# LeeBY68/Hier-SLAM

Measured on AMD Instinct MI355X. Metric: fwd+bwd renders/sec @1200x680, 500k Gaussians, 4-level tree; grad max-abs-err vs ref, higher is better.
Workload: dtype f32; 1 GPU; semantic fwd+bwd render, 1200x680, P=500000 slam Gaussians, K=26 semantic channels, dense upstream grads on colour/semantic/depth/median/opacity; P=500000, visible=480888, num_rendered=1136056, width=1200, height=680, K=26, parallelism=single GPU, keyframes_per_rank=1

## Files before the change

### hier-slam_amd/csrc/hsr_api.hip

```cpp
#include <stdarg.h>

#include <chrono>
#include <time.h>
#include <stdio.h>
#include <stdlib.h>
#include <string.h>

#include <mutex>
#include <type_traits>
#include <vector>

#include "../../include/hsr_rasterizer.h"
#include "hsr_tile_common.h"

namespace {

thread_local char g_err[512] = "";

template <typename T>
inline void take(char*& p, T*& out, size_t count)
{
    uintptr_t a = (reinterpret_cast<uintptr_t>(p) + 255) & ~(uintptr_t)255;
    out = reinterpret_cast<T*>(a);
    p = reinterpret_cast<char*>(out + count);
// ... 134 lines not shown
    if (d < 0 || d >= HSR_MAX_DEVICES) {
        hsr_set_error("device index %d out of range", d);
        return HSR_ERR_INVALID_ARGUMENT;
    }
    g_pc = &g_counters_by_device[d];
    if (!g_pinned) {
        HSR_HIP_CHECK(hipHostMalloc(reinterpret_cast<void**>(&g_pinned), 64, hipHostMallocPortable | hipHostMallocMapped));
        g_pinned[0] = g_pinned[1] = g_pinned[2] = 0;
        HSR_HIP_CHECK(hipHostGetDevicePointer(reinterpret_cast<void**>(&g_pinned_dev), g_pinned, 0));
    }
    return HSR_OK;
}
int read_counter_begin(const uint32_t* dev, hipStream_t stream)
{
    int rc;
    if ((rc = counter_buffer()) != HSR_OK) return rc;
    if (!g_counter_event) HSR_HIP_CHECK(hipEventCreateWithFlags(&g_counter_event, hipEventDisableTiming));
    HSR_HIP_CHECK(hipMemcpyAsync(g_pinned, dev, sizeof(uint32_t), hipMemcpyDeviceToHost, stream));
    HSR_HIP_CHECK(hipMemcpyAsync(g_pinned + 2, dev + 1, sizeof(uint32_t), hipMemcpyDeviceToHost, stream));
    HSR_HIP_CHECK(hipEventRecord(g_counter_event, stream));
    return HSR_OK;
}
thread_local double g_host_wait_ms = 0.0;
thread_local int g_last_per_tile = 0;
int read_counter_end(uint32_t* host_out)
{
    const auto t0 = std::chrono::steady_clock::now();
    HSR_HIP_CHECK(hipEventSynchronize(g_counter_event));
    g_host_wait_ms += std::chrono::duration<double, std::milli>(std::chrono::steady_clock::now() - t0).count();
    *host_out = g_pinned[0];
    return HSR_OK;
}
int poll_counter(uint32_t seq, hipStream_t stream, uint32_t* host_out, volatile uint32_t* slot = nullptr)
{
    const auto t0 = std::chrono::steady_clock::now();
    if (slot) {
        unsigned spins = 0;
        uint32_t cur;
        while ((cur = __atomic_load_n(&slot[1], __ATOMIC_ACQUIRE)) != seq) {
            if (cur != 0 && (int32_t)(cur - seq) > 0) {
                hsr_set_error("non-blocking forward: this call's num_rendered was overwritten — more than %d non-blocking forwards were "
                              "started on the device before it was resolved (resolve or drop earlier ones first)", HSR_ASYNC_SLOTS - 1);
                return HSR_ERR_INVALID_ARGUMENT;
            }
            if ((++spins & 0xFFFu) == 0) {
                const double el = std::chrono::duration<double>(std::chrono::steady_clock::now() - t0).count();
                if (el > 10.0) {
// ... 169 lines not shown
            seq = ++g_counter_seq;
            if (seq == 0) seq = ++g_counter_seq;
            slot_dev = g_pinned_dev;
        }
        StageTimer tm(HSR_STAGE_FWD_DUPLICATE, stream);
        hsr_launch_bin_count(plan, P, radii, tiles_x, tiles_y, g, bin_scratch, im.ranges, stream, slot_dev, seq);
    } else {
        StageTimer tm(HSR_STAGE_FWD_SCAN, stream);
        hsr_launch_scan_block_sums(P, g, stream);
    }
    HSR_LAUNCH_CHECK(in.debug, stream);

    if (!binned && (rc = read_counter_begin(g.counters, stream)) != HSR_OK) return rc;

    RenderFwdArgs ra;
    ra.W = W; ra.H = H; ra.K = in.semantic ? in.K : 0; ra.semantic = in.semantic;
    ra.ranges = im.ranges; ra.point_list = nullptr; ra.masks = nullptr; ra.means2D = g.means2D; ra.conic_opacity = g.conic_opacity;
    ra.depths = g.depths; ra.colors = in.colors_precomp ? in.colors_precomp : g.rgb; ra.semantics = in.semantics;
    ra.rec = g.rec;
    ra.final_T = im.final_T; ra.n_contrib = im.n_contrib; ra.median_pos = im.median_pos;
    ra.out_color = in.out_color; ra.out_semantic = in.out_semantic; ra.out_depth = in.out_depth;
    ra.out_median_depth = in.out_median; ra.out_opacity = in.out_opacity; ra.out_mask = in.out_mask;
    ra.bin = BinDevRef{nullptr, nullptr, 0};
    if (!in.semantic && !in.out_mask) {
        hsr_set_error("out_mask is NULL");
        return HSR_ERR_INVALID_ARGUMENT;
    }

    bool speculated = false;
    if (will_speculate) {
        const BinDevRef ref{static_cast<char*>(binning->ptr), reinterpret_cast<const uint32_t*>(g.counters), binning->capacity};
        BinState none{nullptr, nullptr, nullptr, nullptr, nullptr};
        {
            StageTimer tm(HSR_STAGE_FWD_DUPLICATE, stream);
            hsr_launch_bin_emit(plan, P, radii, tiles_x, tiles_y, g, bin_scratch, im.ranges, nullptr, stream, &ref);
        }
        {
            StageTimer tm(HSR_STAGE_FWD_SORT, stream);
            hsr_launch_tile_sort(none, T, P, im.ranges, stream, &ref, g_last_per_tile);
        }
        ra.bin = ref;
        {
            StageTimer tm(HSR_STAGE_FWD_RENDER, stream);
            hsr_launch_render_forward(ra, stream);
        }
        HSR_HIP_CHECK(hipGetLastError());
        speculated = true;
    }
    if (go_async) {
        ticket->seq = seq;
        ticket->device = slot_device;
        ticket->slot = slot_host;
        ticket->binning_base = static_cast<char*>(binning->ptr);
        ticket->binning_capacity = binning->capacity;
        ticket->prefiltered = in.prefiltered;
        return HSR_PENDING;
    }

    uint32_t R32 = 0;
    if ((rc = binned ? poll_counter(seq, stream, &R32) : read_counter_end(&R32)) != HSR_OK) return rc;
    if (R32 > 0x7fffffffu) {
        hsr_set_error("num_rendered %u overflows int", R32);
        return HSR_ERR_INVALID_ARGUMENT;
    }
    const int R = (int)R32;
    if (in.prefiltered && __atomic_load_n(&g_pinned[2], __ATOMIC_RELAXED) != 0) {
        hsr_set_error("Point is filtered although prefiltered is set. This shouldn't happen!");
        return HSR_ERR_INVALID_ARGUMENT;
    }
    if (speculated) {
        BinState chk;
        const BinDevRef ref{static_cast<char*>(binning->ptr), nullptr, binning->capacity};
        g_last_per_tile = R / (T > 0 ? T : 1);
        if (hsr_bin_resolve(ref, R32, &chk)) return R;
        hsr_launch_bin_count(plan, P, radii, tiles_x, tiles_y, g, bin_scratch, im.ranges, stream, g_pinned_dev, seq);
        ra.bin = BinDevRef{nullptr, nullptr, 0};
    }

    char* bptr;
    if ((rc = acquire(binning, hsr_required_binning_bytes(R), "binning", &bptr)) != HSR_OK) return rc;
    BinState b;
    hsr_carve_bin(bptr, R, &b);

    if (binned) {
        StageTimer tm(HSR_STAGE_FWD_DUPLICATE, stream);
        hsr_launch_bin_emit(plan, P, radii, tiles_x, tiles_y, g, bin_scratch, im.ranges, b.keys, stream);
    }
    if (binned) {
        HSR_LAUNCH_CHECK(in.debug, stream);
        StageTimer tm(HSR_STAGE_FWD_SORT, stream);
        if (R > 0) hsr_launch_tile_sort(b, T, P, im.ranges, stream, nullptr, R / (T > 0 ? T : 1));
    } else {
        const bool emit_sorted = hsr_sort_emit_into_sorted_buffers(end_bit);
        uint64_t* emit_k = emit_sorted ? b.keys : b.keys_unsorted;
        uint32_t* emit_v = emit_sorted ? b.vals : b.vals_unsorted;
        {
            StageTimer tm(HSR_STAGE_FWD_DUPLICATE, stream);
            BinState be = b;
            be.keys_unsorted = emit_k;
            be.vals_unsorted = emit_v;
            hsr_launch_duplicate(P, radii, tiles_x, tiles_y, g, be, im.ranges, stream);
        }
        HSR_LAUNCH_CHECK(in.debug, stream);
        StageTimer tm(HSR_STAGE_FWD_SORT, stream);
        if ((rc = hsr_launch_sort_pairs(b, R, end_bit, T, im.ranges, stream)) != HSR_OK) return rc;
    }
    HSR_LAUNCH_CHECK(in.debug, stream);

    ra.point_list = b.vals;
    ra.masks = b.vals_unsorted;
    {
        StageTimer tm(HSR_STAGE_FWD_RENDER, stream);
        hsr_launch_render_forward(ra, stream);
    }
// ... 480 lines not shown
```

### hier-slam_amd/csrc/hsr_common.h

```cpp
#pragma once
#include <hip/hip_runtime.h>
#include <stddef.h>
#include <stdint.h>

#define HSR_TILE_X 16
#define HSR_TILE_Y 16
#define HSR_TILE_PIX 256
#define HSR_NUM_CHANNELS 3

struct GeomState {
    float* depths;
    float2* means2D;
    float4* conic_opacity;
    float* cov3D;
    float* rgb;
    uint8_t* clamped;
    uint32_t* tiles_touched;
    uint32_t* point_offsets;
    int* radii;
    uint32_t* block_sums;
    uint32_t* counters;
    float4* rec;
};
struct ImgState {
// ... 68 lines not shown
    const float* colors_precomp;
    const float* viewmatrix;
    const float* projmatrix;
    const float* cam_pos;
    float tan_fovx, tan_fovy, focal_x, focal_y;
    int* radii;
    int prefiltered;
    int tiles_x, tiles_y;
};

int hsr_launch_mark_visible(int P, const float* means3D, const float* view, const float* proj, uint8_t* present,
                            hipStream_t stream);
int hsr_launch_preprocess(const PreprocessArgs& a, GeomState& g, hipStream_t stream);
int hsr_launch_scan_block_sums(int P, GeomState& g, hipStream_t stream);
int hsr_launch_duplicate(int P, const int* radii, int tiles_x, int tiles_y, GeomState& g, BinState& b, uint2* ranges,
                         hipStream_t stream);
int hsr_launch_sort_pairs(BinState& b, int R, int end_bit, int T, uint2* ranges, hipStream_t stream);
struct HsrBinPlan { int nblk, per_block; };
bool hsr_bin_plan(int P, int T, size_t scratch_words, HsrBinPlan* plan);
int hsr_launch_bin_count(const HsrBinPlan& plan, int P, const int* radii, int tiles_x, int tiles_y, GeomState& g, uint32_t* scratch,
                         uint2* ranges, hipStream_t stream, uint32_t* host_counter = nullptr, uint32_t host_seq = 0);
int hsr_launch_bin_emit(const HsrBinPlan& plan, int P, const int* radii, int tiles_x, int tiles_y, GeomState& g, const uint32_t* scratch,
                        uint2* ranges, uint64_t* comp, hipStream_t stream, const BinDevRef* ref = nullptr);
int hsr_launch_tile_sort(BinState& b, int T, int P, const uint2* ranges, hipStream_t stream, const BinDevRef* ref = nullptr,
                         int avg_per_tile_hint = 0);
int hsr_sort_tile_passes(int end_bit);
bool hsr_sort_emit_into_sorted_buffers(int end_bit);
int hsr_launch_tile_ranges(int R, int T, const uint64_t* keys, uint2* ranges, hipStream_t stream);
int hsr_launch_tile_ranges_only(int R, const uint64_t* keys, uint2* ranges, hipStream_t stream);

struct RenderFwdArgs {
    int W, H, K, semantic;
    const uint2* ranges;
    const uint32_t* point_list;
    uint32_t* masks;
    const float2* means2D;
    const float4* conic_opacity;
    const float* depths;
    const float* colors;
    const float4* rec;
    const float* semantics;
    float* final_T;
    uint32_t* n_contrib;
    uint32_t* median_pos;
    float* out_color;
    float* out_semantic;
    float* out_depth;
    float* out_median_depth;
    float* out_opacity;
    float* out_mask;
    BinDevRef bin;
};
int hsr_launch_render_forward(const RenderFwdArgs& a, hipStream_t stream);

struct RenderBwdArgs {
    int W, H, K, semantic, P;
    const float* bg;
    const uint2* ranges;
// ... 75 lines not shown
```

### hier-slam_amd/csrc/hsr_render_fwd.hip

```cpp

#include "hsr_tile_common.h"

#ifdef HSR_TRACE
__device__ unsigned long long g_hsr_trace_fwd[16384 * 8];
extern "C" int hsr_debug_read_trace_fwd(unsigned long long* host, int n)
{
    return (int)hipMemcpyFromSymbol(host, HIP_SYMBOL(g_hsr_trace_fwd), sizeof(unsigned long long) * (size_t)n);
}
#define TRF_NOW() clock64()
#define TRF_ADD(acc, t0) (acc) += (unsigned long long)(clock64() - (t0))
#else
#define TRF_NOW() 0ll
#define TRF_ADD(acc, t0) ((void)0)
#endif

namespace {

template <int W>
__device__ __forceinline__ void quad_fma_words(float (&s)[16], const float (&x)[4], float w)
{
    static_assert(W >= 1 && W <= 4, "1..4 words = 4..16 channels per block");
    if constexpr (W == 4) {
        asm("s_nop 1\n\t"
            "v_fmac_f32_dpp %0, %16, %20 quad_perm:[0,0,0,0] row_mask:0xf bank_mask:0xf\n\t"
// ... 43 lines not shown
            : "+v"(s[0]), "+v"(s[1]), "+v"(s[2]), "+v"(s[3]), "+v"(s[4]), "+v"(s[5]), "+v"(s[6]), "+v"(s[7])
            : "v"(x[0]), "v"(x[1]), "v"(w));
    } else {
        asm("s_nop 1\n\t"
            "v_fmac_f32_dpp %0, %4, %5 quad_perm:[0,0,0,0] row_mask:0xf bank_mask:0xf\n\t"
            "v_fmac_f32_dpp %1, %4, %5 quad_perm:[1,1,1,1] row_mask:0xf bank_mask:0xf\n\t"
            "v_fmac_f32_dpp %2, %4, %5 quad_perm:[2,2,2,2] row_mask:0xf bank_mask:0xf\n\t"
            "v_fmac_f32_dpp %3, %4, %5 quad_perm:[3,3,3,3] row_mask:0xf bank_mask:0xf"
            : "+v"(s[0]), "+v"(s[1]), "+v"(s[2]), "+v"(s[3])
            : "v"(x[0]), "v"(w));
    }
}

template <int KC, bool BASE, bool MASK, bool ALIGNED, bool PF = false>
__global__ void __launch_bounds__(256, KC <= 26 ? (KC == 16 ? 5 : 4) : (PF ? (KC <= 48 ? 4 : (KC <= 80 ? 3 : 2)) : 1)) render_fwd_kernel(RenderFwdArgs a, int c0)
{
    constexpr int BATCH = KC <= 32 ? (KC > 26 ? 200 : 240)
                                   : (KC <= 48 ? 152 : ((KC <= 64 || KC == 74) ? 144 : (KC <= 80 ? 136 : (KC <= 112 ? 144 : 128))));
    static_assert(KC <= 32 || PF, "batch sizes beyond 32 channels assume the touched rows (PF)");
    constexpr int RW = (KC + 2 + 3) & ~3;
    constexpr bool QS = PF && KC > 0;
    constexpr int NGF = QS ? RW / 16 : 0;
    constexpr int REM = QS ? (RW % 16) / 4 : 0;
    __shared__ float4 s_rec[BATCH * 2];
    __shared__ float4 s_row[BATCH * (RW / 4)];
    __shared__ uint8_t s_sublist[16 * HSR_SUB_LSTRIDE];
    __shared__ uint8_t s_subcnt[4][16];
    __shared__ int s_wdone[4];

    const int tile = hsr_block_tile(blockIdx.x, ((a.W + HSR_TILE_X - 1) / HSR_TILE_X) * ((a.H + HSR_TILE_Y - 1) / HSR_TILE_Y));
    if (tile >= ((a.W + HSR_TILE_X - 1) / HSR_TILE_X) * ((a.H + HSR_TILE_Y - 1) / HSR_TILE_Y)) return;
    const int t = threadIdx.x, wv = t >> 6;
    if (a.bin.base) {
        BinState bs;
        if (!hsr_bin_resolve(a.bin, *a.bin.R_dev, &bs)) {
            hsr_poison_tile(a, tile, t, BASE, c0, KC);
            return;
        }
        a.point_list = bs.vals;
        a.masks = bs.vals_unsorted;
    }
    const TileGeom tg = tile_geom_sub(tile, a.W, a.H, t);
    const bool inside = tg.inside;
    const size_t N = (size_t)a.W * a.H;
    float pfx = tg.pfx, pfy = tg.pfy;
    asm volatile("" : "+v"(pfx), "+v"(pfy));
    const float tile_x0 = (float)(tg.tx * HSR_TILE_X), tile_y0 = (float)(tg.ty * HSR_TILE_Y);

    unsigned long long tr_bar = 0, tr_stage = 0, tr_blend = 0, tr_iters = 0, tr_pub = 0;
    (void)tr_pub;
    const long long tr_t0 = TRF_NOW();
    long long tr_t1 = tr_t0;
    (void)tr_bar; (void)tr_stage; (void)tr_blend; (void)tr_iters; (void)tr_t0; (void)tr_t1;
    const uint2 range = a.ranges[tile];
    const int n = (int)(range.y - range.x);

    float T = 1.0f;
    uint32_t last_contributor = 0;
    float C0 = 0, C1 = 0, C2 = 0, Dd = 0, Mm = 0;
    uint32_t median_at = 0;
    float median_D = 15.0f;
    float S[KC > 0 ? KC : 1];
#pragma unroll
    for (int c = 0; c < (KC > 0 ? KC : 1); c++) S[c] = 0.f;
    bool done = !inside;

    int id_next = 0;
    float2 p_xy = {0, 0};
    float4 p_co = {0, 0, 0, 0};
    float p_r = 0, p_g = 0, p_b = 0, p_d = 0;
    float p_sem[(KC > 0 && !PF) ? KC : 1];
#pragma unroll
    for (int c = 0; c < ((KC > 0 && !PF) ? KC : 1); c++) p_sem[c] = 0.f;
    constexpr int NPF = PF ? (KC + 15) / 16 + 1 : 1;
    float pf_t[NPF];
#pragma unroll
    for (int c = 0; c < NPF; c++) pf_t[c] = 0.f;
    float pf_sink = 0.f;
// ... 16 lines not shown
            if (KC > 0 && PF) {
                const float* row = a.semantics + id * (size_t)a.K + c0;
                const int last = min(KC, a.K - c0) - 1;
#pragma unroll
                for (int c = 0; c < NPF; c++) pf_t[c] = row[min(16 * c, last)];
            } else if (KC > 0) {
                if (ALIGNED) {
                    const float2* row = reinterpret_cast<const float2*>(a.semantics + id * (size_t)KC);
#pragma unroll
                    for (int q = 0; q < KC / 2; q++) {
                        const float2 v = row[q];
                        p_sem[PF ? 0 : 2 * q] = v.x;
                        p_sem[PF ? 0 : 2 * q + 1] = v.y;
                    }
                } else {
                    const float* row = a.semantics + id * (size_t)a.K + c0;
#pragma unroll
                    for (int c = 0; c < KC; c++) p_sem[PF ? 0 : c] = (c0 + c < a.K) ? row[c] : 0.f;
                }
            }
        }
    };
    if (n > 0) {
        const int id0 = fetch_id(0);
        id_next = fetch_id(BATCH);
        load_record(id0);
    }
    auto resolve_median = [&](int start) {
        if (BASE && median_at > (uint32_t)start) {
            const int j = (int)median_at - 1 - start;
            constexpr int c = KC + 1;
            constexpr int pos = (QS && c / 16 < NGF) ? (16 * (c / 16) + 4 * (c % 4) + (c % 16) / 4) : c;
            median_D = reinterpret_cast<const float*>(s_row)[j * RW + pos];
        }
    };


    for (int start = 0; start < n; start += BATCH) {
        const bool wave_done = __ballot(!done) == 0ull;
        if ((t & 63) == 0) s_wdone[wv] = wave_done;
        const long long tb0 = TRF_NOW();
        (void)tb0;
        __syncthreads();
        TRF_ADD(tr_bar, tb0);
        if (start == 0) tr_t1 = TRF_NOW();
        const long long ts0 = TRF_NOW();
        (void)ts0;
        if (s_wdone[0] & s_wdone[1] & s_wdone[2] & s_wdone[3]) break;
// ... 282 lines not shown
```

### hier-slam_amd/csrc/hsr_sort.hip

```cpp
#include "hsr_common.h"

namespace {

constexpr int SORT_THREADS = 256;
constexpr int SORT_ITEMS = 16;
constexpr int SORT_TILE = SORT_THREADS * SORT_ITEMS;
static_assert(SORT_TILE == HSR_SORT_TILE, "hsr_common.h sizes the histogram scratch");

__global__ void __launch_bounds__(SORT_THREADS) sort_hist_kernel(const uint64_t* __restrict__ keys, int n, int shift,
                                                                 uint32_t mask, int nblocks, uint32_t* __restrict__ hist)
{
    __shared__ uint32_t h[256];
    h[threadIdx.x] = 0;
    __syncthreads();
    const int base = blockIdx.x * SORT_TILE;
#pragma unroll 4
    for (int i = 0; i < SORT_ITEMS; i++) {
        const int j = base + i * SORT_THREADS + threadIdx.x;
        if (j < n) atomicAdd(&h[(uint32_t)(keys[j] >> shift) & mask], 1u);
    }
    __syncthreads();
    hist[(size_t)threadIdx.x * nblocks + blockIdx.x] = h[threadIdx.x];
}

// ... 86 lines not shown
        wcnt[0][threadIdx.x] = g;
        wcnt[1][threadIdx.x] = g + c0;
        wcnt[2][threadIdx.x] = g + c0 + c1;
        wcnt[3][threadIdx.x] = g + c0 + c1 + c2;
    }
    __syncthreads();
#pragma unroll
    for (int r = 0; r < SORT_ITEMS; r++) {
        const int j = base + r * 64 + lane;
        if (j < n) {
            const uint32_t d = (uint32_t)(key[r] >> shift) & mask;
            const uint32_t pos = wcnt[w][d] + rank[r];
            kout[pos] = key[r];
            vout[pos] = val[r];
        }
    }
}

}

uint32_t hsr_sort_hist_entries(int R) { return hsr_sort_hist_entries_inline((uint32_t)(R > 0 ? R : 0)); }


constexpr int TS_MAX = 2048;

__device__ __forceinline__ void ts_block_radix(uint64_t* ka, uint32_t* va, uint64_t* kb, uint32_t* vb, int r0, int n,
                                               uint32_t* hist , uint32_t (*wcnt)[256], int gid_passes)
{
    const int t = threadIdx.x, lane = t & 63, w = t >> 6;
    const uint64_t lt = (1ull << lane) - 1ull;
    const int npass = gid_passes + 4;
    for (int pass = 0; pass < npass; pass++) {
        const bool on_gid = pass < gid_passes;
        const int shift = 8 * (on_gid ? pass : pass - gid_passes);
        hist[t] = 0;
#pragma unroll
        for (int i = 0; i < 4; i++) wcnt[i][t] = 0;
        __syncthreads();
        for (int i = t; i < n; i += 256)
            atomicAdd(&hist[((on_gid ? va[r0 + i] : (uint32_t)ka[r0 + i]) >> shift) & 255u], 1u);
        __syncthreads();
        {
            const uint32_t v = hist[t];
            uint32_t inc = v;
#pragma unroll
            for (int o = 1; o < 64; o <<= 1) {
                const uint32_t x = __shfl_up(inc, o);
                if (lane >= o) inc += x;
            }
            __shared__ uint32_t wt[4];
            if (lane == 63) wt[w] = inc;
            __syncthreads();
            uint32_t off = 0;
#pragma unroll
            for (int i = 0; i < 4; i++) off += i < w ? wt[i] : 0u;
            hist[t] = off + inc - v;
        }
        __syncthreads();
        for (int c = 0; c < n; c += 256) {
            const int i = c + t;
            const bool valid = i < n;
            const uint64_t k = valid ? ka[r0 + i] : 0ull;
            const uint32_t v = valid ? va[r0 + i] : 0u;
            const uint32_t d = ((on_gid ? v : (uint32_t)k) >> shift) & 255u;
            uint64_t m = __ballot(valid);
#pragma unroll
            for (int b = 0; b < 8; b++) {
                const bool bit = (d >> b) & 1u;
                const uint64_t bal = __ballot(bit);
                m &= bit ? bal : ~bal;
            }
            const uint32_t before = __popcll(m & lt);
            if (valid && before == 0) wcnt[w][d] = (uint32_t)__popcll(m);
            __syncthreads();
            if (valid) {
                uint32_t pos = hist[d] + before;
#pragma unroll
                for (int i2 = 0; i2 < 4; i2++) pos += i2 < w ? wcnt[i2][d] : 0u;
                kb[r0 + pos] = k;
                vb[r0 + pos] = v;
            }
            __syncthreads();
            hist[t] += wcnt[0][t] + wcnt[1][t] + wcnt[2][t] + wcnt[3][t];
#pragma unroll
            for (int i2 = 0; i2 < 4; i2++) wcnt[i2][t] = 0;
            __syncthreads();
        }
        uint64_t* tk = ka; ka = kb; kb = tk;
        uint32_t* tv = va; va = vb; vb = tv;
        __threadfence_block();
    }
    if (npass & 1) {
        __syncthreads();
        for (int i = t; i < n; i += 256) {
            kb[r0 + i] = ka[r0 + i];
            vb[r0 + i] = va[r0 + i];
        }
    }
}

constexpr int TP_MAX = 1024;
constexpr int TQ_MAX = 2048;

template <int E, int NT>
__device__ __forceinline__ void net_bitonic(uint64_t (&x)[E], int tid, ulonglong2* buf)
{
    constexpr int N = NT * E;
#pragma unroll
    for (int k = 2; k <= N; k <<= 1) {
#pragma unroll
        for (int j = k >> 1; j > 0; j >>= 1) {
            if (j < E) {
#pragma unroll
                for (int r = 0; r < E; r++) {
                    if ((r & j) == 0) {
                        const bool up = k < E ? ((r & k) == 0) : (((E * tid) & k) == 0);
                        const uint64_t a = x[r], b = x[r + j];
                        const bool sw = (a > b) == up;
                        x[r] = sw ? b : a;
                        x[r + j] = sw ? a : b;
                    }
                }
            } else {
                const int m = j / E;
                const bool cross = m >= 64;
#pragma unroll
                for (int q = 0; q < E / 2; q++) buf[q * NT + tid] = make_ulonglong2(x[2 * q], x[2 * q + 1]);
                if (cross) {
                    __syncthreads();
                } else {
                    __builtin_amdgcn_fence(__ATOMIC_RELEASE, "wavefront");
                    __builtin_amdgcn_wave_barrier();
                    __builtin_amdgcn_fence(__ATOMIC_ACQUIRE, "wavefront");
                }
                const bool keep_min = ((tid & m) == 0) == (((E * tid) & k) == 0);
#pragma unroll
                for (int q = 0; q < E / 2; q++) {
                    const ulonglong2 y = buf[q * NT + (tid ^ m)];
                    const uint64_t a0 = x[2 * q], a1 = x[2 * q + 1];
                    x[2 * q] = keep_min ? (a0 < y.x ? a0 : y.x) : (a0 > y.x ? a0 : y.x);
                    x[2 * q + 1] = keep_min ? (a1 < y.y ? a1 : y.y) : (a1 > y.y ? a1 : y.y);
                }
                if (cross) {
                    __syncthreads();
                } else {
                    __builtin_amdgcn_fence(__ATOMIC_RELEASE, "wavefront");
                    __builtin_amdgcn_wave_barrier();
                    __builtin_amdgcn_fence(__ATOMIC_ACQUIRE, "wavefront");
                }
            }
        }
    }
}

__device__ __forceinline__ void block_sort_tile(int tile, const uint2* __restrict__ ranges, uint64_t* __restrict__ keys,
                                                uint32_t* __restrict__ vals, uint64_t* __restrict__ keys_alt,
                                                uint32_t* __restrict__ vals_alt, int gid_passes, int composite_in, uint64_t* comp,
                                                uint32_t* hist, uint32_t (*wcnt)[256])
{
    const uint2 rg = ranges[tile];
    const int r0 = (int)rg.x, n = (int)(rg.y - rg.x);
    const int t = threadIdx.x;
    const uint64_t my_tile_hi = (uint64_t)tile << 32;
    if (n <= 0) return;
    if (n == 1 || n > TS_MAX) {
        if (composite_in) {
            for (int i = t; i < n; i += 256) {
                const uint64_t c = keys[r0 + i];
                keys[r0 + i] = my_tile_hi | (c >> 32);
                vals[r0 + i] = (uint32_t)c;
            }
            __syncthreads();
        }
        if (n == 1) return;
    }
    if (n > TS_MAX) {
        ts_block_radix(keys, vals, keys_alt, vals_alt, r0, n, hist, wcnt, gid_passes);
        return;
    }
    if (composite_in) {
        static_assert(TQ_MAX == TS_MAX && TS_MAX * 8 >= 4 * 256 * 16, "exchange buffer = the LDS network's key array");
        uint64_t x[8];
#pragma unroll
        for (int r = 0; r < 8; r++) {
            const int e = 8 * t + r;
            x[r] = e < n ? keys[r0 + e] : ~0ull;
        }
        net_bitonic<8, 256>(x, t, reinterpret_cast<ulonglong2*>(comp));
#pragma unroll
        for (int r = 0; r < 8; r++) {
            const int e = 8 * t + r;
            if (e < n) {
                keys[r0 + e] = my_tile_hi | (x[r] >> 32);
                vals[r0 + e] = (uint32_t)x[r];
            }
        }
        return;
    }
    int N = 64;
    while (N < n) N <<= 1;
    const uint64_t tile_hi = keys[r0] & 0xFFFFFFFF00000000ull;
    for (int i = t; i < N; i += 256)
        comp[i] = i < n ? (((keys[r0 + i] & 0xFFFFFFFFull) << 32) | (uint64_t)vals[r0 + i]) : ~0ull;
    __syncthreads();
    bool cross = false;
    for (int k = 2; k <= N; k <<= 1) {
        for (int j = k >> 1; j > 0; j >>= 1) {
            if (j >= 128 || cross) __syncthreads();
            cross = j >= 128;
            for (int i = t; i < N / 2; i += 256) {
                const int lo = ((i & ~(j - 1)) << 1) | (i & (j - 1));
                const int hi = lo | j;
                const bool up = (lo & k) == 0;
                const uint64_t a = comp[lo], b = comp[hi];
                if ((a > b) == up) {
                    comp[lo] = b;
                    comp[hi] = a;
                }
            }
        }
    }
    __syncthreads();
    for (int i = t; i < n; i += 256) {
        const uint64_t c = comp[i];
        keys[r0 + i] = tile_hi | (c >> 32);
        vals[r0 + i] = (uint32_t)c;
    }
}

__global__ void __launch_bounds__(256) tile_sort_kernel(const uint2* __restrict__ ranges, uint64_t* __restrict__ keys,
                                                        uint32_t* __restrict__ vals, uint64_t* __restrict__ keys_alt,
                                                        uint32_t* __restrict__ vals_alt, int gid_passes, int composite_in, BinDevRef ref)
{
    if (ref.base) {
        BinState bs;
        if (!hsr_bin_resolve(ref, *ref.R_dev, &bs)) return;
        keys = bs.keys; vals = bs.vals; keys_alt = bs.keys_unsorted; vals_alt = bs.vals_unsorted;
    }
    __shared__ uint64_t comp[TS_MAX];
    __shared__ uint32_t hist[256];
    __shared__ uint32_t wcnt[4][256];
    if (composite_in == 2) {
        const uint2 rg = ranges[blockIdx.x];
        if (rg.y - rg.x <= (uint32_t)TP_MAX) return;
        composite_in = 1;
    }
    block_sort_tile((int)blockIdx.x, ranges, keys, vals, keys_alt, vals_alt, gid_passes, composite_in, comp, hist, wcnt);
}

template <int E>
__device__ __forceinline__ void pair_sort_tile(int r0, int n, int tid, uint64_t tile_hi, uint64_t* __restrict__ keys,
                                               uint32_t* __restrict__ vals, ulonglong2* buf)
{
    uint64_t x[E];
#pragma unroll
    for (int r = 0; r < E; r++) {
        const int e = E * tid + r;
        x[r] = e < n ? keys[r0 + e] : ~0ull;
    }
    net_bitonic<E, 128>(x, tid, buf);
#pragma unroll
    for (int r = 0; r < E; r++) {
        const int e = E * tid + r;
        if (e < n) {
            keys[r0 + e] = tile_hi | (x[r] >> 32);
            vals[r0 + e] = (uint32_t)x[r];
        }
    }
}

__global__ void __launch_bounds__(256, 7) tile_sort_pair_kernel(int T, const uint2* __restrict__ ranges, uint64_t* __restrict__ keys,
                                                             uint32_t* __restrict__ vals, uint64_t* __restrict__ keys_alt,
                                                             uint32_t* __restrict__ vals_alt, int gid_passes, int big_too, BinDevRef ref)
{
    constexpr int RAW_WG = TS_MAX * 8 + 256 * 4 + 4 * 256 * 4, RAW_PAIR = 2 * 4 * 128 * 16;
    constexpr int RAW = RAW_WG > RAW_PAIR ? RAW_WG : RAW_PAIR;
    __shared__ __attribute__((aligned(16))) unsigned char s_raw[RAW];
    __shared__ int s_big[2];
    if (ref.base) {
        BinState bs;
        if (!hsr_bin_resolve(ref, *ref.R_dev, &bs)) return;
        keys = bs.keys; vals = bs.vals; keys_alt = bs.keys_unsorted; vals_alt = bs.vals_unsorted;
    }
    const int pair = threadIdx.x >> 7, tid = threadIdx.x & 127;
    const int tile = blockIdx.x * 2 + pair;
    int n = 0, r0 = 0;
    if (tile < T) {
        const uint2 rg = ranges[tile];
        r0 = (int)rg.x;
        n = (int)(rg.y - rg.x);
    }
    if (tid == 0) s_big[pair] = n > TP_MAX;
    {
        ulonglong2* buf = reinterpret_cast<ulonglong2*>(s_raw) + pair * (4 * 128);
        const uint64_t tile_hi = (uint64_t)tile << 32;
        if (n > 0 && n <= 256) pair_sort_tile<2>(r0, n, tid, tile_hi, keys, vals, buf);
        else if (n > 256 && n <= 512) pair_sort_tile<4>(r0, n, tid, tile_hi, keys, vals, buf);
        else if (n > 512 && n <= TP_MAX) pair_sort_tile<8>(r0, n, tid, tile_hi, keys, vals, buf);
        else { __syncthreads(); __syncthreads(); }
    }
    if (!big_too) return;
    __syncthreads();
    uint64_t* comp = reinterpret_cast<uint64_t*>(s_raw);
    uint32_t* hist = reinterpret_cast<uint32_t*>(s_raw + TS_MAX * 8);
    uint32_t (*wcnt)[256] = reinterpret_cast<uint32_t (*)[256]>(s_raw + TS_MAX * 8 + 256 * 4);
    for (int w = 0; w < 2; w++) {
        if (!s_big[w]) continue;
        block_sort_tile(blockIdx.x * 2 + w, ranges, keys, vals, keys_alt, vals_alt, gid_passes, 1, comp, hist, wcnt);
        __syncthreads();
    }
}

int hsr_sort_tile_passes(int end_bit)
{
    const int tile_bits = end_bit - 32;
    return tile_bits <= 0 ? 0 : (tile_bits + 7) / 8;
}
bool hsr_sort_emit_into_sorted_buffers(int end_bit) { return (hsr_sort_tile_passes(end_bit) & 1) == 0; }

int hsr_launch_sort_pairs(BinState& b, int R, int end_bit, int T, uint2* ranges, hipStream_t stream)
{
    if (R <= 0) return HSR_OK;
    const int passes = hsr_sort_tile_passes(end_bit);
    const int tile_bits = end_bit - 32;
    const int nblocks = (R + SORT_TILE - 1) / SORT_TILE;
    uint32_t* totals = b.hist + (size_t)256 * nblocks;
    uint64_t* ka = (passes & 1) ? b.keys_unsorted : b.keys;
    uint32_t* va = (passes & 1) ? b.vals_unsorted : b.vals;
    uint64_t* kb = (passes & 1) ? b.keys : b.keys_unsorted;
    uint32_t* vb = (passes & 1) ? b.vals : b.vals_unsorted;
    const int bits_per_pass = passes ? (tile_bits + passes - 1) / passes : 0;
    for (int p = 0; p < passes; p++) {
        const int shift = 32 + bits_per_pass * p;
        const int bits = min(bits_per_pass, end_bit - shift);
        const uint32_t mask = (1u << bits) - 1u;
        sort_hist_kernel<<<nblocks, SORT_THREADS, 0, stream>>>(ka, R, shift, mask, nblocks, b.hist);
        sort_rowscan_kernel<<<256, 64, 0, stream>>>(b.hist, nblocks, totals);
        sort_scatter_kernel<<<nblocks, SORT_THREADS, 0, stream>>>(ka, va, kb, vb, R, shift, mask, nblocks, b.hist, totals);
        uint64_t* tk = ka; ka = kb; kb = tk;
        uint32_t* tv = va; va = vb; vb = tv;
    }
    hsr_launch_tile_ranges_only(R, b.keys, ranges, stream);
    tile_sort_kernel<<<T, 256, 0, stream>>>(ranges, b.keys, b.vals, b.keys_unsorted, b.vals_unsorted, 0, 0, BinDevRef{nullptr, nullptr, 0});
    return HSR_OK;
}

int hsr_launch_tile_sort(BinState& b, int T, int P, const uint2* ranges, hipStream_t stream, const BinDevRef* ref, int avg_per_tile_hint)
{
    int bits = 0;
    while (bits < 32 && (1ull << bits) < (unsigned long long)(P > 1 ? P : 1)) bits++;
    const BinDevRef r = ref ? *ref : BinDevRef{nullptr, nullptr, 0};
    const bool many_big = avg_per_tile_hint > 800;
    tile_sort_pair_kernel<<<(T + 1) / 2, 256, 0, stream>>>(T, ranges, b.keys, b.vals, b.keys_unsorted, b.vals_unsorted, (bits + 7) / 8,
                                                           many_big ? 0 : 1, r);
    if (many_big)
        tile_sort_kernel<<<T, 256, 0, stream>>>(ranges, b.keys, b.vals, b.keys_unsorted, b.vals_unsorted, (bits + 7) / 8, 2, r);
    return HSR_OK;
}
```

Measured before the change: 1753 renders/s.

## Fuse per-tile sort into forward render kernel and stage sorted ids in LDS

Removes the separate tile-sort kernel launch on the binned and speculative paths. The render-forward kernel now sorts its own tile's keys at its start, using bitonic networks for small tiles and block radix for large ones, and reuses the staging LDS buffer as the exchange space. Sorted point ids are also written into LDS so the first batches are fetched without a global reload. This trades a kernel launch and a global round trip for extra LDS pressure and sort work inside the render kernel, which may lower occupancy and serialize the sort with rendering per tile.

```diff
diff --git a/hier-slam_amd/csrc/hsr_api.hip b/hier-slam_amd/csrc/hsr_api.hip
--- a/hier-slam_amd/csrc/hsr_api.hip
+++ b/hier-slam_amd/csrc/hsr_api.hip
@@ -180,7 +180,6 @@
     return HSR_OK;
 }
 thread_local double g_host_wait_ms = 0.0;
-thread_local int g_last_per_tile = 0;
 int read_counter_end(uint32_t* host_out)
 {
     const auto t0 = std::chrono::steady_clock::now();
@@ -396,6 +395,7 @@
     ra.out_color = in.out_color; ra.out_semantic = in.out_semantic; ra.out_depth = in.out_depth;
     ra.out_median_depth = in.out_median; ra.out_opacity = in.out_opacity; ra.out_mask = in.out_mask;
     ra.bin = BinDevRef{nullptr, nullptr, 0};
+    ra.sort = 0; ra.sort_gid_passes = hsr_tile_sort_gid_passes(P); ra.keys = nullptr; ra.keys_alt = nullptr;
     if (!in.semantic && !in.out_mask) {
         hsr_set_error("out_mask is NULL");
         return HSR_ERR_INVALID_ARGUMENT;
@@ -404,16 +404,12 @@
     bool speculated = false;
     if (will_speculate) {
         const BinDevRef ref{static_cast<char*>(binning->ptr), reinterpret_cast<const uint32_t*>(g.counters), binning->capacity};
-        BinState none{nullptr, nullptr, nullptr, nullptr, nullptr};
         {
             StageTimer tm(HSR_STAGE_FWD_DUPLICATE, stream);
             hsr_launch_bin_emit(plan, P, radii, tiles_x, tiles_y, g, bin_scratch, im.ranges, nullptr, stream, &ref);
         }
-        {
-            StageTimer tm(HSR_STAGE_FWD_SORT, stream);
-            hsr_launch_tile_sort(none, T, P, im.ranges, stream, &ref, g_last_per_tile);
-        }
         ra.bin = ref;
+        ra.sort = 1;
         {
             StageTimer tm(HSR_STAGE_FWD_RENDER, stream);
             hsr_launch_render_forward(ra, stream);
@@ -445,7 +441,6 @@
     if (speculated) {
         BinState chk;
         const BinDevRef ref{static_cast<char*>(binning->ptr), nullptr, binning->capacity};
-        g_last_per_tile = R / (T > 0 ? T : 1);
         if (hsr_bin_resolve(ref, R32, &chk)) return R;
         hsr_launch_bin_count(plan, P, radii, tiles_x, tiles_y, g, bin_scratch, im.ranges, stream, g_pinned_dev, seq);
         ra.bin = BinDevRef{nullptr, nullptr, 0};
@@ -461,9 +456,9 @@
         hsr_launch_bin_emit(plan, P, radii, tiles_x, tiles_y, g, bin_scratch, im.ranges, b.keys, stream);
     }
     if (binned) {
-        HSR_LAUNCH_CHECK(in.debug, stream);
-        StageTimer tm(HSR_STAGE_FWD_SORT, stream);
-        if (R > 0) hsr_launch_tile_sort(b, T, P, im.ranges, stream, nullptr, R / (T > 0 ? T : 1));
+        ra.sort = 1;
+        ra.keys = b.keys;
+        ra.keys_alt = b.keys_unsorted;
     } else {
         const bool emit_sorted = hsr_sort_emit_into_sorted_buffers(end_bit);
         uint64_t* emit_k = emit_sorted ? b.keys : b.keys_unsorted;
diff --git a/hier-slam_amd/csrc/hsr_common.h b/hier-slam_amd/csrc/hsr_common.h
--- a/hier-slam_amd/csrc/hsr_common.h
+++ b/hier-slam_amd/csrc/hsr_common.h
@@ -114,8 +114,12 @@
                          uint2* ranges, hipStream_t stream, uint32_t* host_counter = nullptr, uint32_t host_seq = 0);
 int hsr_launch_bin_emit(const HsrBinPlan& plan, int P, const int* radii, int tiles_x, int tiles_y, GeomState& g, const uint32_t* scratch,
                         uint2* ranges, uint64_t* comp, hipStream_t stream, const BinDevRef* ref = nullptr);
-int hsr_launch_tile_sort(BinState& b, int T, int P, const uint2* ranges, hipStream_t stream, const BinDevRef* ref = nullptr,
-                         int avg_per_tile_hint = 0);
+__host__ __device__ inline int hsr_tile_sort_gid_passes(int P)
+{
+    int bits = 0;
+    while (bits < 32 && (1ull << bits) < (unsigned long long)(P > 1 ? P : 1)) bits++;
+    return (bits + 7) / 8;
+}
 int hsr_sort_tile_passes(int end_bit);
 bool hsr_sort_emit_into_sorted_buffers(int end_bit);
 int hsr_launch_tile_ranges(int R, int T, const uint64_t* keys, uint2* ranges, hipStream_t stream);
@@ -124,8 +128,12 @@
 struct RenderFwdArgs {
     int W, H, K, semantic;
     const uint2* ranges;
-    const uint32_t* point_list;
+    uint32_t* point_list;
     uint32_t* masks;
+    int sort;
+    int sort_gid_passes;
+    uint64_t* keys;
+    uint64_t* keys_alt;
     const float2* means2D;
     const float4* conic_opacity;
     const float* depths;
diff --git a/hier-slam_amd/csrc/hsr_render_fwd.hip b/hier-slam_amd/csrc/hsr_render_fwd.hip
--- a/hier-slam_amd/csrc/hsr_render_fwd.hip
+++ b/hier-slam_amd/csrc/hsr_render_fwd.hip
@@ -1,5 +1,6 @@
 
 #include "hsr_tile_common.h"
+#include "hsr_tile_sort.h"
 
 #ifdef HSR_TRACE
 __device__ unsigned long long g_hsr_trace_fwd[16384 * 8];
@@ -89,8 +90,13 @@
     constexpr bool QS = PF && KC > 0;
     constexpr int NGF = QS ? RW / 16 : 0;
     constexpr int REM = QS ? (RW % 16) / 4 : 0;
-    __shared__ float4 s_rec[BATCH * 2];
-    __shared__ float4 s_row[BATCH * (RW / 4)];
+    constexpr int STAGE_F4 = BATCH * 2 + BATCH * (RW / 4);
+    constexpr int NID = BATCH + 256;
+    constexpr bool NET8 = STAGE_F4 * 16 >= 16384 + 4 * NID;
+    static_assert(!BASE || STAGE_F4 * 16 >= 8192 + 4 * NID, "the in-kernel tile sort needs 8 KB + the ids of LDS");
+    __shared__ float4 s_stage[STAGE_F4];
+    float4* const s_rec = s_stage;
+    float4* const s_row = s_stage + BATCH * 2;
     __shared__ uint8_t s_sublist[16 * HSR_SUB_LSTRIDE];
     __shared__ uint8_t s_subcnt[4][16];
     __shared__ int s_wdone[4];
@@ -106,6 +112,8 @@
         }
         a.point_list = bs.vals;
         a.masks = bs.vals_unsorted;
+        a.keys = bs.keys;
+        a.keys_alt = bs.keys_unsorted;
     }
     const TileGeom tg = tile_geom_sub(tile, a.W, a.H, t);
     const bool inside = tg.inside;
@@ -121,6 +129,12 @@
     (void)tr_bar; (void)tr_stage; (void)tr_blend; (void)tr_iters; (void)tr_t0; (void)tr_t1;
     const uint2 range = a.ranges[tile];
     const int n = (int)(range.y - range.x);
+    bool ids_lds = false;
+    if constexpr (BASE) {
+        if (a.sort && c0 == 0)
+            ids_lds = fused_sort_tile<NET8>(tile, (int)range.x, n, a.keys, a.point_list, a.keys_alt, a.masks, a.sort_gid_passes,
+                                            reinterpret_cast<unsigned char*>(s_stage), min(n, NID));
+    }
 
     float T = 1.0f;
     uint32_t last_contributor = 0;
@@ -183,8 +197,9 @@
         }
     };
     if (n > 0) {
-        const int id0 = fetch_id(0);
-        id_next = fetch_id(BATCH);
+        const uint32_t* s_ids = reinterpret_cast<const uint32_t*>(reinterpret_cast<const unsigned char*>(s_stage) + (NET8 ? 16384 : 8192));
+        const int id0 = ids_lds ? (int)s_ids[min(t, n - 1)] : fetch_id(0);
+        id_next = ids_lds ? (int)s_ids[min(BATCH + t, n - 1)] : fetch_id(BATCH);
         load_record(id0);
     }
     auto resolve_median = [&](int start) {
diff --git a/hier-slam_amd/csrc/hsr_sort.hip b/hier-slam_amd/csrc/hsr_sort.hip
--- a/hier-slam_amd/csrc/hsr_sort.hip
+++ b/hier-slam_amd/csrc/hsr_sort.hip
@@ -1,4 +1,4 @@
-#include "hsr_common.h"
+#include "hsr_tile_sort.h"
 
 namespace {
 
@@ -132,293 +132,14 @@
 uint32_t hsr_sort_hist_entries(int R) { return hsr_sort_hist_entries_inline((uint32_t)(R > 0 ? R : 0)); }
 
 
-constexpr int TS_MAX = 2048;
-
-__device__ __forceinline__ void ts_block_radix(uint64_t* ka, uint32_t* va, uint64_t* kb, uint32_t* vb, int r0, int n,
-                                               uint32_t* hist , uint32_t (*wcnt)[256], int gid_passes)
-{
-    const int t = threadIdx.x, lane = t & 63, w = t >> 6;
-    const uint64_t lt = (1ull << lane) - 1ull;
-    const int npass = gid_passes + 4;
-    for (int pass = 0; pass < npass; pass++) {
-        const bool on_gid = pass < gid_passes;
-        const int shift = 8 * (on_gid ? pass : pass - gid_passes);
-        hist[t] = 0;
-#pragma unroll
-        for (int i = 0; i < 4; i++) wcnt[i][t] = 0;
-        __syncthreads();
-        for (int i = t; i < n; i += 256)
-            atomicAdd(&hist[((on_gid ? va[r0 + i] : (uint32_t)ka[r0 + i]) >> shift) & 255u], 1u);
-        __syncthreads();
-        {
-            const uint32_t v = hist[t];
-            uint32_t inc = v;
-#pragma unroll
-            for (int o = 1; o < 64; o <<= 1) {
-                const uint32_t x = __shfl_up(inc, o);
-                if (lane >= o) inc += x;
-            }
-            __shared__ uint32_t wt[4];
-            if (lane == 63) wt[w] = inc;
-            __syncthreads();
-            uint32_t off = 0;
-#pragma unroll
-            for (int i = 0; i < 4; i++) off += i < w ? wt[i] : 0u;
-            hist[t] = off + inc - v;
-        }
-        __syncthreads();
-        for (int c = 0; c < n; c += 256) {
-            const int i = c + t;
-            const bool valid = i < n;
-            const uint64_t k = valid ? ka[r0 + i] : 0ull;
-            const uint32_t v = valid ? va[r0 + i] : 0u;
-            const uint32_t d = ((on_gid ? v : (uint32_t)k) >> shift) & 255u;
-            uint64_t m = __ballot(valid);
-#pragma unroll
-            for (int b = 0; b < 8; b++) {
-                const bool bit = (d >> b) & 1u;
-                const uint64_t bal = __ballot(bit);
-                m &= bit ? bal : ~bal;
-            }
-            const uint32_t before = __popcll(m & lt);
-            if (valid && before == 0) wcnt[w][d] = (uint32_t)__popcll(m);
-            __syncthreads();
-            if (valid) {
-                uint32_t pos = hist[d] + before;
-#pragma unroll
-                for (int i2 = 0; i2 < 4; i2++) pos += i2 < w ? wcnt[i2][d] : 0u;
-                kb[r0 + pos] = k;
-                vb[r0 + pos] = v;
-            }
-            __syncthreads();
-            hist[t] += wcnt[0][t] + wcnt[1][t] + wcnt[2][t] + wcnt[3][t];
-#pragma unroll
-            for (int i2 = 0; i2 < 4; i2++) wcnt[i2][t] = 0;
-            __syncthreads();
-        }
-        uint64_t* tk = ka; ka = kb; kb = tk;
-        uint32_t* tv = va; va = vb; vb = tv;
-        __threadfence_block();
-    }
-    if (npass & 1) {
-        __syncthreads();
-        for (int i = t; i < n; i += 256) {
-            kb[r0 + i] = ka[r0 + i];
-            vb[r0 + i] = va[r0 + i];
-        }
-    }
-}
-
-constexpr int TP_MAX = 1024;
-constexpr int TQ_MAX = 2048;
-
-template <int E, int NT>
-__device__ __forceinline__ void net_bitonic(uint64_t (&x)[E], int tid, ulonglong2* buf)
-{
-    constexpr int N = NT * E;
-#pragma unroll
-    for (int k = 2; k <= N; k <<= 1) {
-#pragma unroll
-        for (int j = k >> 1; j > 0; j >>= 1) {
-            if (j < E) {
-#pragma unroll
-                for (int r = 0; r < E; r++) {
-                    if ((r & j) == 0) {
-                        const bool up = k < E ? ((r & k) == 0) : (((E * tid) & k) == 0);
-                        const uint64_t a = x[r], b = x[r + j];
-                        const bool sw = (a > b) == up;
-                        x[r] = sw ? b : a;
-                        x[r + j] = sw ? a : b;
-                    }
-                }
-            } else {
-                const int m = j / E;
-                const bool cross = m >= 64;
-#pragma unroll
-                for (int q = 0; q < E / 2; q++) buf[q * NT + tid] = make_ulonglong2(x[2 * q], x[2 * q + 1]);
-                if (cross) {
-                    __syncthreads();
-                } else {
-                    __builtin_amdgcn_fence(__ATOMIC_RELEASE, "wavefront");
-                    __builtin_amdgcn_wave_barrier();
-                    __builtin_amdgcn_fence(__ATOMIC_ACQUIRE, "wavefront");
-                }
-                const bool keep_min = ((tid & m) == 0) == (((E * tid) & k) == 0);
-#pragma unroll
-                for (int q = 0; q < E / 2; q++) {
-                    const ulonglong2 y = buf[q * NT + (tid ^ m)];
-                    const uint64_t a0 = x[2 * q], a1 = x[2 * q + 1];
-                    x[2 * q] = keep_min ? (a0 < y.x ? a0 : y.x) : (a0 > y.x ? a0 : y.x);
-                    x[2 * q + 1] = keep_min ? (a1 < y.y ? a1 : y.y) : (a1 > y.y ? a1 : y.y);
-                }
-                if (cross) {
-                    __syncthreads();
-                } else {
-                    __builtin_amdgcn_fence(__ATOMIC_RELEASE, "wavefront");
-                    __builtin_amdgcn_wave_barrier();
-                    __builtin_amdgcn_fence(__ATOMIC_ACQUIRE, "wavefront");
-                }
-            }
-        }
-    }
-}
-
-__device__ __forceinline__ void block_sort_tile(int tile, const uint2* __restrict__ ranges, uint64_t* __restrict__ keys,
-                                                uint32_t* __restrict__ vals, uint64_t* __restrict__ keys_alt,
-                                                uint32_t* __restrict__ vals_alt, int gid_passes, int composite_in, uint64_t* comp,
-                                                uint32_t* hist, uint32_t (*wcnt)[256])
-{
-    const uint2 rg = ranges[tile];
-    const int r0 = (int)rg.x, n = (int)(rg.y - rg.x);
-    const int t = threadIdx.x;
-    const uint64_t my_tile_hi = (uint64_t)tile << 32;
-    if (n <= 0) return;
-    if (n == 1 || n > TS_MAX) {
-        if (composite_in) {
-            for (int i = t; i < n; i += 256) {
-                const uint64_t c = keys[r0 + i];
-                keys[r0 + i] = my_tile_hi | (c >> 32);
-                vals[r0 + i] = (uint32_t)c;
-            }
-            __syncthreads();
-        }
-        if (n == 1) return;
-    }
-    if (n > TS_MAX) {
-        ts_block_radix(keys, vals, keys_alt, vals_alt, r0, n, hist, wcnt, gid_passes);
-        return;
-    }
-    if (composite_in) {
-        static_assert(TQ_MAX == TS_MAX && TS_MAX * 8 >= 4 * 256 * 16, "exchange buffer = the LDS network's key array");
-        uint64_t x[8];
-#pragma unroll
-        for (int r = 0; r < 8; r++) {
-            const int e = 8 * t + r;
-            x[r] = e < n ? keys[r0 + e] : ~0ull;
-        }
-        net_bitonic<8, 256>(x, t, reinterpret_cast<ulonglong2*>(comp));
-#pragma unroll
-        for (int r = 0; r < 8; r++) {
-            const int e = 8 * t + r;
-            if (e < n) {
-                keys[r0 + e] = my_tile_hi | (x[r] >> 32);
-                vals[r0 + e] = (uint32_t)x[r];
-            }
-        }
-        return;
-    }
-    int N = 64;
-    while (N < n) N <<= 1;
-    const uint64_t tile_hi = keys[r0] & 0xFFFFFFFF00000000ull;
-    for (int i = t; i < N; i += 256)
-        comp[i] = i < n ? (((keys[r0 + i] & 0xFFFFFFFFull) << 32) | (uint64_t)vals[r0 + i]) : ~0ull;
-    __syncthreads();
-    bool cross = false;
-    for (int k = 2; k <= N; k <<= 1) {
-        for (int j = k >> 1; j > 0; j >>= 1) {
-            if (j >= 128 || cross) __syncthreads();
-            cross = j >= 128;
-            for (int i = t; i < N / 2; i += 256) {
-                const int lo = ((i & ~(j - 1)) << 1) | (i & (j - 1));
-                const int hi = lo | j;
-                const bool up = (lo & k) == 0;
-                const uint64_t a = comp[lo], b = comp[hi];
-                if ((a > b) == up) {
-                    comp[lo] = b;
-                    comp[hi] = a;
-                }
-            }
-        }
-    }
-    __syncthreads();
-    for (int i = t; i < n; i += 256) {
-        const uint64_t c = comp[i];
-        keys[r0 + i] = tile_hi | (c >> 32);
-        vals[r0 + i] = (uint32_t)c;
-    }
-}
-
 __global__ void __launch_bounds__(256) tile_sort_kernel(const uint2* __restrict__ ranges, uint64_t* __restrict__ keys,
                                                         uint32_t* __restrict__ vals, uint64_t* __restrict__ keys_alt,
-                                                        uint32_t* __restrict__ vals_alt, int gid_passes, int composite_in, BinDevRef ref)
+                                                        uint32_t* __restrict__ vals_alt)
 {
-    if (ref.base) {
-        BinState bs;
-        if (!hsr_bin_resolve(ref, *ref.R_dev, &bs)) return;
-        keys = bs.keys; vals = bs.vals; keys_alt = bs.keys_unsorted; vals_alt = bs.vals_unsorted;
-    }
     __shared__ uint64_t comp[TS_MAX];
     __shared__ uint32_t hist[256];
     __shared__ uint32_t wcnt[4][256];
-    if (composite_in == 2) {
-        const uint2 rg = ranges[blockIdx.x];
-        if (rg.y - rg.x <= (uint32_t)TP_MAX) return;
-        composite_in = 1;
-    }
-    block_sort_tile((int)blockIdx.x, ranges, keys, vals, keys_alt, vals_alt, gid_passes, composite_in, comp, hist, wcnt);
-}
-
-template <int E>
-__device__ __forceinline__ void pair_sort_tile(int r0, int n, int tid, uint64_t tile_hi, uint64_t* __restrict__ keys,
-                                               uint32_t* __restrict__ vals, ulonglong2* buf)
-{
-    uint64_t x[E];
-#pragma unroll
-    for (int r = 0; r < E; r++) {
-        const int e = E * tid + r;
-        x[r] = e < n ? keys[r0 + e] : ~0ull;
-    }
-    net_bitonic<E, 128>(x, tid, buf);
-#pragma unroll
-    for (int r = 0; r < E; r++) {
-        const int e = E * tid + r;
-        if (e < n) {
-            keys[r0 + e] = tile_hi | (x[r] >> 32);
-            vals[r0 + e] = (uint32_t)x[r];
-        }
-    }
-}
-
-__global__ void __launch_bounds__(256, 7) tile_sort_pair_kernel(int T, const uint2* __restrict__ ranges, uint64_t* __restrict__ keys,
-                                                             uint32_t* __restrict__ vals, uint64_t* __restrict__ keys_alt,
-                                                             uint32_t* __restrict__ vals_alt, int gid_passes, int big_too, BinDevRef ref)
-{
-    constexpr int RAW_WG = TS_MAX * 8 + 256 * 4 + 4 * 256 * 4, RAW_PAIR = 2 * 4 * 128 * 16;
-    constexpr int RAW = RAW_WG > RAW_PAIR ? RAW_WG : RAW_PAIR;
-    __shared__ __attribute__((aligned(16))) unsigned char s_raw[RAW];
-    __shared__ int s_big[2];
-    if (ref.base) {
-        BinState bs;
-        if (!hsr_bin_resolve(ref, *ref.R_dev, &bs)) return;
-        keys = bs.keys; vals = bs.vals; keys_alt = bs.keys_unsorted; vals_alt = bs.vals_unsorted;
-    }
-    const int pair = threadIdx.x >> 7, tid = threadIdx.x & 127;
-    const int tile = blockIdx.x * 2 + pair;
-    int n = 0, r0 = 0;
-    if (tile < T) {
-        const uint2 rg = ranges[tile];
-        r0 = (int)rg.x;
-        n = (int)(rg.y - rg.x);
-    }
-    if (tid == 0) s_big[pair] = n > TP_MAX;
-    {
-        ulonglong2* buf = reinterpret_cast<ulonglong2*>(s_raw) + pair * (4 * 128);
-        const uint64_t tile_hi = (uint64_t)tile << 32;
-        if (n > 0 && n <= 256) pair_sort_tile<2>(r0, n, tid, tile_hi, keys, vals, buf);
-        else if (n > 256 && n <= 512) pair_sort_tile<4>(r0, n, tid, tile_hi, keys, vals, buf);
-        else if (n > 512 && n <= TP_MAX) pair_sort_tile<8>(r0, n, tid, tile_hi, keys, vals, buf);
-        else { __syncthreads(); __syncthreads(); }
-    }
-    if (!big_too) return;
-    __syncthreads();
-    uint64_t* comp = reinterpret_cast<uint64_t*>(s_raw);
-    uint32_t* hist = reinterpret_cast<uint32_t*>(s_raw + TS_MAX * 8);
-    uint32_t (*wcnt)[256] = reinterpret_cast<uint32_t (*)[256]>(s_raw + TS_MAX * 8 + 256 * 4);
-    for (int w = 0; w < 2; w++) {
-        if (!s_big[w]) continue;
-        block_sort_tile(blockIdx.x * 2 + w, ranges, keys, vals, keys_alt, vals_alt, gid_passes, 1, comp, hist, wcnt);
-        __syncthreads();
-    }
+    block_sort_tile((int)blockIdx.x, ranges, keys, vals, keys_alt, vals_alt, comp, hist, wcnt);
 }
 
 int hsr_sort_tile_passes(int end_bit)
@@ -451,19 +172,6 @@
         uint32_t* tv = va; va = vb; vb = tv;
     }
     hsr_launch_tile_ranges_only(R, b.keys, ranges, stream);
-    tile_sort_kernel<<<T, 256, 0, stream>>>(ranges, b.keys, b.vals, b.keys_unsorted, b.vals_unsorted, 0, 0, BinDevRef{nullptr, nullptr, 0});
+    tile_sort_kernel<<<T, 256, 0, stream>>>(ranges, b.keys, b.vals, b.keys_unsorted, b.vals_unsorted);
     return HSR_OK;
 }
-
-int hsr_launch_tile_sort(BinState& b, int T, int P, const uint2* ranges, hipStream_t stream, const BinDevRef* ref, int avg_per_tile_hint)
-{
-    int bits = 0;
-    while (bits < 32 && (1ull << bits) < (unsigned long long)(P > 1 ? P : 1)) bits++;
-    const BinDevRef r = ref ? *ref : BinDevRef{nullptr, nullptr, 0};
-    const bool many_big = avg_per_tile_hint > 800;
-    tile_sort_pair_kernel<<<(T + 1) / 2, 256, 0, stream>>>(T, ranges, b.keys, b.vals, b.keys_unsorted, b.vals_unsorted, (bits + 7) / 8,
-                                                           many_big ? 0 : 1, r);
-    if (many_big)
-        tile_sort_kernel<<<T, 256, 0, stream>>>(ranges, b.keys, b.vals, b.keys_unsorted, b.vals_unsorted, (bits + 7) / 8, 2, r);
-    return HSR_OK;
-}
diff --git a/hier-slam_amd/csrc/hsr_tile_sort.h b/hier-slam_amd/csrc/hsr_tile_sort.h
--- /dev/null
+++ b/hier-slam_amd/csrc/hsr_tile_sort.h
@@ -0,0 +1,234 @@
+#pragma once
+#include "hsr_common.h"
+
+constexpr int TS_MAX = 2048;
+
+__device__ __forceinline__ void ts_block_radix(uint64_t* ka, uint32_t* va, uint64_t* kb, uint32_t* vb, int r0, int n,
+                                               uint32_t* hist , uint32_t (*wcnt)[256], int gid_passes)
+{
+    const int t = threadIdx.x, lane = t & 63, w = t >> 6;
+    const uint64_t lt = (1ull << lane) - 1ull;
+    const int npass = gid_passes + 4;
+    for (int pass = 0; pass < npass; pass++) {
+        const bool on_gid = pass < gid_passes;
+        const int shift = 8 * (on_gid ? pass : pass - gid_passes);
+        hist[t] = 0;
+#pragma unroll
+        for (int i = 0; i < 4; i++) wcnt[i][t] = 0;
+        __syncthreads();
+        for (int i = t; i < n; i += 256)
+            atomicAdd(&hist[((on_gid ? va[r0 + i] : (uint32_t)ka[r0 + i]) >> shift) & 255u], 1u);
+        __syncthreads();
+        {
+            const uint32_t v = hist[t];
+            uint32_t inc = v;
+#pragma unroll
+            for (int o = 1; o < 64; o <<= 1) {
+                const uint32_t x = __shfl_up(inc, o);
+                if (lane >= o) inc += x;
+            }
+            __shared__ uint32_t wt[4];
+            if (lane == 63) wt[w] = inc;
+            __syncthreads();
+            uint32_t off = 0;
+#pragma unroll
+            for (int i = 0; i < 4; i++) off += i < w ? wt[i] : 0u;
+            hist[t] = off + inc - v;
+        }
+        __syncthreads();
+        for (int c = 0; c < n; c += 256) {
+            const int i = c + t;
+            const bool valid = i < n;
+            const uint64_t k = valid ? ka[r0 + i] : 0ull;
+            const uint32_t v = valid ? va[r0 + i] : 0u;
+            const uint32_t d = ((on_gid ? v : (uint32_t)k) >> shift) & 255u;
+            uint64_t m = __ballot(valid);
+#pragma unroll
+            for (int b = 0; b < 8; b++) {
+                const bool bit = (d >> b) & 1u;
+                const uint64_t bal = __ballot(bit);
+                m &= bit ? bal : ~bal;
+            }
+            const uint32_t before = __popcll(m & lt);
+            if (valid && before == 0) wcnt[w][d] = (uint32_t)__popcll(m);
+            __syncthreads();
+            if (valid) {
+                uint32_t pos = hist[d] + before;
+#pragma unroll
+                for (int i2 = 0; i2 < 4; i2++) pos += i2 < w ? wcnt[i2][d] : 0u;
+                kb[r0 + pos] = k;
+                vb[r0 + pos] = v;
+            }
+            __syncthreads();
+            hist[t] += wcnt[0][t] + wcnt[1][t] + wcnt[2][t] + wcnt[3][t];
+#pragma unroll
+            for (int i2 = 0; i2 < 4; i2++) wcnt[i2][t] = 0;
+            __syncthreads();
+        }
+        uint64_t* tk = ka; ka = kb; kb = tk;
+        uint32_t* tv = va; va = vb; vb = tv;
+        __threadfence_block();
+    }
+    if (npass & 1) {
+        __syncthreads();
+        for (int i = t; i < n; i += 256) {
+            kb[r0 + i] = ka[r0 + i];
+            vb[r0 + i] = va[r0 + i];
+        }
+    }
+}
+
+
+template <int E, int NT>
+__device__ __forceinline__ void net_bitonic(uint64_t (&x)[E], int tid, ulonglong2* buf)
+{
+    constexpr int N = NT * E;
+#pragma unroll
+    for (int k = 2; k <= N; k <<= 1) {
+#pragma unroll
+        for (int j = k >> 1; j > 0; j >>= 1) {
+            if (j < E) {
+#pragma unroll
+                for (int r = 0; r < E; r++) {
+                    if ((r & j) == 0) {
+                        const bool up = k < E ? ((r & k) == 0) : (((E * tid) & k) == 0);
+                        const uint64_t a = x[r], b = x[r + j];
+                        const bool sw = (a > b) == up;
+                        x[r] = sw ? b : a;
+                        x[r + j] = sw ? a : b;
+                    }
+                }
+            } else {
+                const int m = j / E;
+                const bool cross = m >= 64;
+#pragma unroll
+                for (int q = 0; q < E / 2; q++) buf[q * NT + tid] = make_ulonglong2(x[2 * q], x[2 * q + 1]);
+                if (cross) {
+                    __syncthreads();
+                } else {
+                    __builtin_amdgcn_fence(__ATOMIC_RELEASE, "wavefront");
+                    __builtin_amdgcn_wave_barrier();
+                    __builtin_amdgcn_fence(__ATOMIC_ACQUIRE, "wavefront");
+                }
+                const bool keep_min = ((tid & m) == 0) == (((E * tid) & k) == 0);
+#pragma unroll
+                for (int q = 0; q < E / 2; q++) {
+                    const ulonglong2 y = buf[q * NT + (tid ^ m)];
+                    const uint64_t a0 = x[2 * q], a1 = x[2 * q + 1];
+                    x[2 * q] = keep_min ? (a0 < y.x ? a0 : y.x) : (a0 > y.x ? a0 : y.x);
+                    x[2 * q + 1] = keep_min ? (a1 < y.y ? a1 : y.y) : (a1 > y.y ? a1 : y.y);
+                }
+                if (cross) {
+                    __syncthreads();
+                } else {
+                    __builtin_amdgcn_fence(__ATOMIC_RELEASE, "wavefront");
+                    __builtin_amdgcn_wave_barrier();
+                    __builtin_amdgcn_fence(__ATOMIC_ACQUIRE, "wavefront");
+                }
+            }
+        }
+    }
+}
+
+__device__ __forceinline__ void block_sort_tile(int tile, const uint2* __restrict__ ranges, uint64_t* __restrict__ keys,
+                                                uint32_t* __restrict__ vals, uint64_t* __restrict__ keys_alt,
+                                                uint32_t* __restrict__ vals_alt, uint64_t* comp, uint32_t* hist, uint32_t (*wcnt)[256])
+{
+    const uint2 rg = ranges[tile];
+    const int r0 = (int)rg.x, n = (int)(rg.y - rg.x);
+    const int t = threadIdx.x;
+    if (n <= 1) return;
+    if (n > TS_MAX) {
+        ts_block_radix(keys, vals, keys_alt, vals_alt, r0, n, hist, wcnt, 0);
+        return;
+    }
+    int N = 64;
+    while (N < n) N <<= 1;
+    const uint64_t tile_hi = keys[r0] & 0xFFFFFFFF00000000ull;
+    for (int i = t; i < N; i += 256)
+        comp[i] = i < n ? (((keys[r0 + i] & 0xFFFFFFFFull) << 32) | (uint64_t)vals[r0 + i]) : ~0ull;
+    __syncthreads();
+    bool cross = false;
+    for (int k = 2; k <= N; k <<= 1) {
+        for (int j = k >> 1; j > 0; j >>= 1) {
+            if (j >= 128 || cross) __syncthreads();
+            cross = j >= 128;
+            for (int i = t; i < N / 2; i += 256) {
+                const int lo = ((i & ~(j - 1)) << 1) | (i & (j - 1));
+                const int hi = lo | j;
+                const bool up = (lo & k) == 0;
+                const uint64_t a = comp[lo], b = comp[hi];
+                if ((a > b) == up) {
+                    comp[lo] = b;
+                    comp[hi] = a;
+                }
+            }
+        }
+    }
+    __syncthreads();
+    for (int i = t; i < n; i += 256) {
+        const uint64_t c = comp[i];
+        keys[r0 + i] = tile_hi | (c >> 32);
+        vals[r0 + i] = (uint32_t)c;
+    }
+}
+
+
+constexpr int TP_MAX = 1024;
+template <int E>
+__device__ __forceinline__ void wg_sort_tile(int r0, int n, uint64_t tile_hi, uint64_t* __restrict__ keys, uint32_t* __restrict__ vals,
+                                             ulonglong2* buf, uint32_t* ids, int nid)
+{
+    const int t = threadIdx.x;
+    uint64_t x[E];
+#pragma unroll
+    for (int r = 0; r < E; r++) {
+        const int e = E * t + r;
+        x[r] = e < n ? keys[r0 + e] : ~0ull;
+    }
+    net_bitonic<E, 256>(x, t, buf);
+#pragma unroll
+    for (int r = 0; r < E; r++) {
+        const int e = E * t + r;
+        if (e < n) {
+            keys[r0 + e] = tile_hi | (x[r] >> 32);
+            vals[r0 + e] = (uint32_t)x[r];
+            if (e < nid) ids[e] = (uint32_t)x[r];
+        }
+    }
+}
+
+template <bool NET8>
+__device__ __forceinline__ bool fused_sort_tile(int tile, int r0, int n, uint64_t* __restrict__ keys, uint32_t* __restrict__ vals,
+                                                uint64_t* __restrict__ keys_alt, uint32_t* __restrict__ vals_alt, int gid_passes,
+                                                unsigned char* lds, int nid)
+{
+    constexpr int XB = NET8 ? 16384 : 8192;
+    ulonglong2* buf = reinterpret_cast<ulonglong2*>(lds);
+    uint32_t* ids = reinterpret_cast<uint32_t*>(lds + XB);
+    const uint64_t tile_hi = (uint64_t)tile << 32;
+    bool in_lds = true;
+    if (n <= 0) {
+    } else if (n <= 512) {
+        wg_sort_tile<2>(r0, n, tile_hi, keys, vals, buf, ids, nid);
+    } else if (n <= TP_MAX) {
+        wg_sort_tile<4>(r0, n, tile_hi, keys, vals, buf, ids, nid);
+    } else if (NET8 && n <= TS_MAX) {
+        wg_sort_tile<8>(r0, n, tile_hi, keys, vals, buf, ids, nid);
+    } else {
+        const int t = threadIdx.x;
+        for (int i = t; i < n; i += 256) {
+            const uint64_t c = keys[r0 + i];
+            keys[r0 + i] = tile_hi | (c >> 32);
+            vals[r0 + i] = (uint32_t)c;
+        }
+        __syncthreads();
+        uint32_t* hist = reinterpret_cast<uint32_t*>(lds);
+        uint32_t (*wcnt)[256] = reinterpret_cast<uint32_t (*)[256]>(lds + 256 * 4);
+        ts_block_radix(keys, vals, keys_alt, vals_alt, r0, n, hist, wcnt, gid_passes);
+        __threadfence_block();
+        in_lds = false;
+    }
+    __syncthreads();
+    return in_lds;
+}
```

After: 1779 renders/s (median of 6 runs). About the same (+1.5%).
